# YamaneKoyo/mri-to-speech

Hardware: AMD Instinct MI355X
Metric: rtMRI frames/s end-to-end (256x256 frames -> 64-bin mel -> 11413 Hz wav) (higher is better)
Workload: dtype bf16x3; 1 GPU; e2e rtMRI->wav, 64 clips x 30 frames per GPU at 256x256 (configs[3] per-GPU share); clips_per_gpu=64, frames_per_clip=30, global_batch_clips=64, hw=256, parallelism=dp1, chunk=1920

## Files before the change

### mri-to-speech_amd/csrc/acoustic_cnn.cpp

```cpp
#include <algorithm>
#include <initializer_list>
#include <utility>

#include "plan_util.hpp"
#include "prof.hpp"

namespace m2s {

Acoustic::Acoustic(const StateDict& sd, int n_mels, int hidden, int dtype, int device)
    : dtype_(dtype), device_(device), n_mels_(n_mels), hidden_(hidden) {
  for (auto [name, v] : std::initializer_list<std::pair<const char*, bool*>>{
           {"M2S_IR_FUSED", &ir_fused_},   {"M2S_IR_WS", &ir_ws_},         {"M2S_IR_WS_S2", &ir_ws_s2_},
           {"M2S_IRWS_F32", &irws_f32_},   {"M2S_STEM_FUSED", &stem_fused_}, {"M2S_F8_EXPAND", &f8_expand_},
           {"M2S_F8_S2", &f8_s2_},         {"M2S_F8_ER", &f8_er_},         {"M2S_ER8_X8", &er8_x8_},
           {"M2S_F8_ER2", &f8_er2_},       {"M2S_SE_Y8", &se_y8_},         {"M2S_SE_FUSED", &se_fused_},
           {"M2S_ER_FUSED", &er_fused_},   {"M2S_SE_WS", &se_ws_},         {"M2S_LSTM_PERSISTENT", &lstm_persistent_},
           {"M2S_LSTM_MID", &lstm_mid_},   {"M2S_LSTM_X3", &lstm_x3_},     {"M2S_LSTM_X3G", &lstm_x3g_},
           {"M2S_SE_SP", &se_sp_},         {"M2S_ER_MRG", &er_mrg_},       {"M2S_IR_S2BAND", &ir_s2band_},
           {"M2S_ER_S2_FUSED", &er_s2_fused_}, {"M2S_SEWS_REV", &sews_rev_}})
    env_flag(name, *v);
  env_int("M2S_IRWS_MIN", irws_min_);
  env_int("M2S_SEWS_MIN", sews_min_cus_);
  pack_acoustic(sd, n_mels, hidden, dtype, arena_, p_);
  arena_.upload(device);
  for (auto& b : p_.blocks) {
    b.c1.resolve(arena_);
    if (b.type != 0) b.c2.resolve(arena_);
    if (b.type == 2) {
      b.se1.resolve(arena_);
      b.se2.resolve(arena_);
    }
  }
  p_.lstm_ih.resolve(arena_);
  M2S_HIP(hipHostMalloc(reinterpret_cast<void**>(&err_host_), sizeof(unsigned), hipHostMallocMapped | hipHostMallocCoherent));
  *err_host_ = 0;
  M2S_HIP(hipHostGetDevicePointer(reinterpret_cast<void**>(&err_dev_), err_host_, 0));
  M2S_HIP(hipMalloc(&gsync_, std::max(lstm_small_sync_bytes(), lstm_x3g_sync_bytes())));
}

Acoustic::~Acoustic() {
  if (err_host_) (void)hipHostFree(err_host_);
  if (gsync_) (void)hipFree(gsync_);
}

unsigned Acoustic::take_async_error() { return __atomic_exchange_n(err_host_, 0u, __ATOMIC_ACQ_REL); }

void Acoustic::effnet_dims(int H, int W, size_t* io, size_t* mid, size_t* se) const {
  size_t mio = 0, mmid = 0, mse = 0;
  for_each_backbone_map(H, W, [&](const BlockDef& d, const BlockMap& m) {
    if (d.type == 1) mmid = std::max(mmid, (size_t)m.oh * m.ow * chan_stride(d.mid));
    if (d.type == 2) {
// ... 81 lines not shown
}

template <typename T>
void Acoustic::effnet_cn(EffPass<T>& p, size_t k) {
  const Block& b = p_.blocks[k];
  ConvArgs a = conv2d_args(p, b.c1, p.cur, p.nxt);
  a.act = ACT_SILU;
  a.res = b.skip ? p.cur : nullptr;
  run_conv<T>(a, b.c1, p.s);
}

template <typename T>
void Acoustic::effnet_er(EffPass<T>& p, size_t k) {
  const Block& b = p_.blocks[k];
  const int nc = p.nc, oh = p.oh, ow = p.ow, nh = p.nh, nw = p.nw, qt = p.qt, ql = p.ql;
  T *const cur = p.cur, *const nxt = p.nxt;
  hipStream_t s = p.s;
  const int co = chan_stride(b.cout);
  const double px = (double)nc * nh * nw, flops = 2.0 * px * b.mid * (9.0 * b.cin + b.cout);
  auto unfused = [&] {
    ConvArgs a = conv2d_args(p, b.c1, cur, p.b.M);
    a.act = ACT_SILU;
    ConvArgs q = pw_args(b.c2, p.b.M, nxt, nc * nh * nw, nh * nw);
    q.res = b.skip ? cur : nullptr;
    if (kSplit<T> && er_s2_fused_ && b.stride == 2 && conv_gemm_er_supported(a, q)) {
      launch_conv_gemm_er(a, q, s, flops,
                          4.0 * ((double)nc * oh * ow * b.cin + px * b.cout + (9.0 * b.cin + b.cout) * b.mid));
    } else {
      run_conv<T>(a, b.c1, s);
      run_conv<T>(q, b.c2, s);
    }
  };
  if constexpr (kSplit<T>) {
    if (er_fused_ && b.er_sp && er_sp_supported(nh, nw, b.c1.cs_in, b.mid, co)) {
      launch_er_sp(cur, nc, nh, nw, b.c1.cs_in, b.mid, co, arena_.ptr(b.er_sp_w), b.c1.b, b.c2.b, nxt, flops,
                   4.0 * px * (b.c1.cs_in + co), s, er_mrg_);
    } else if (er_fused_ && b.ers_sp && b.stride == 2 && ers2_sp_supported(nh, nw, b.c1.cs_in, b.mid, co)) {
      launch_ers2_sp(cur, nc, oh, ow, nh, nw, qt, ql, b.c1.cs_in, b.mid, co, arena_.ptr(b.er_wexp), b.c1.b,
                     arena_.ptr(b.er_wpwl), b.c2.b, nxt, flops, 4.0 * ((double)nc * oh * ow * b.c1.cs_in + px * co), s);
    } else {
      unfused();
    }
  } else if constexpr (std::is_same<T, bf16_t>::value) {
    uint8_t *const cur8 = p.cur8, *const *const X8 = p.b.X8, *&next8 = p.next8;
    const Block* const nb = k + 1 < p_.blocks.size() ? &p_.blocks[k + 1] : nullptr;
    uint8_t* const er8_next = X8[0] && f8_er_ && nb && ((er8_x8_ && nb->er8) || (f8_er2_ && nb->er8w))
                                  ? (cur8 == X8[0] ? X8[1] : X8[0])
                                  : nullptr;
    if (er_fused_ && f8_er_ && b.er8 && er8_fused_supported(nh, nw, b.cin, b.mid, b.cout)) {
      uint8_t* y8 = cur8 && er8_next && er8_fused_supported(nh, nw, b.cout, b.mid, b.cout) ? er8_next : nullptr;
      launch_er8_fused(cur, nc, nh, nw, arena_.at<uint8_t>(b.er8_wexp), arena_.at<float>(b.er8_sexp), b.c1.b,
                       arena_.at<uint8_t>(b.er8_wpwl), arena_.at<float>(b.er8_spwl), b.c2.b, nxt, flops,
                       2.0 * px * (2.0 * b.cin) + (3.0 * 8 * 2048 + 2 * 2048), s, cur8, y8);
      next8 = y8;
    } else if (er_fused_ && b.er_frag && er_fused_supported(nh, nw, b.cin, b.mid, b.cout, b.c1.kp, b.c2.kp)) {
      launch_er_fused(cur, nc, nh, nw, arena_.at<bf16_t>(b.er_wexp), b.c1.b, arena_.at<bf16_t>(b.er_wpwl), b.c2.b, nxt,
                      flops, 2.0 * px * (2.0 * b.cin) + 2.0 * (9.0 * 32 * 128 + 128 * 32), s);
    } else if (er_fused_ && f8_er_ && f8_er2_ && b.er8w && cur8 &&
               er8w_fused_supported(nh, nw, b.c1.cs_in, b.mid, b.cout)) {
      uint8_t* y8 = er8_next && nb->er8w ? er8_next : nullptr;
      launch_er8w_fused(cur, cur8, nc, nh, nw, arena_.at<uint8_t>(b.er8w_w), arena_.at<float>(b.er8w_sexp), b.c1.b,
                        arena_.at<float>(b.er8w_spwl), b.c2.b, nxt, y8, flops,
                        px * (b.cin + 2.0 * b.cin + 2.0 * b.cout + (y8 ? b.cout : 0.0)) + (9.0 * b.cin + b.cout) * b.mid, s);
      next8 = y8;
    } else if (er_fused_ && b.er_frag && er2_fused_supported(nh, nw, b.c1.cs_in, b.mid, b.cout, b.c1.kp, b.c2.kp)) {
      launch_er2_fused(cur, nc, nh, nw, arena_.at<bf16_t>(b.er_wexp), b.c1.b, b.c2.b, nxt, flops,
                       2.0 * px * (2.0 * b.c1.cs_in) + 2.0 * er2_stage_elems(), s);
    } else if (er_fused_ && b.er_frag && b.stride == 2 &&
               ers2_fused_supported(nh, nw, b.c1.cs_in, b.mid, co, b.c1.kp, b.c2.kp)) {
// ... 249 lines not shown
```

### mri-to-speech_amd/csrc/er_sp_fused.hip

```cpp
#include <algorithm>

#include "kernels.hpp"
#include "lds_dma.hpp"
#include "prof.hpp"

namespace m2s {
namespace {

__device__ __forceinline__ bf16x8 frag(const char* p) { return *reinterpret_cast<const bf16x8*>(p); }
__device__ __forceinline__ f32x4 mfma(bf16x8 a, bf16x8 b, f32x4 c) {
  return __builtin_amdgcn_mfma_f32_16x16x32_bf16(a, b, c, 0, 0, 0);
}

struct ErSpArgs {
  const bf16_t* x;
  const bf16_t* wst;
  const float* bexp;
  const float* bpwl;
  bf16_t* y;
  int N, H, W, tiles_x, tiles_y;
};

template <int TH, int CSI, int NT, int ON, int NW, int MRG>
__global__ void __launch_bounds__(64 * NW, NW == 4 ? 2 : 1) er_sp_kernel(const ErSpArgs a) {
  constexpr int TW = 16, HW = TW + 2, HH = TH + 2, HPIX = HH * HW;
  constexpr int HPB = (HPIX + 63) / 64;
  constexpr int HPLANE = HPB * 1024;
  constexpr int CH = CSI / 8;
  constexpr int HBUF = 2 * CH * HPLANE;
  constexpr int HP = 2 * CH * HPB / NW;
  static_assert((2 * CH * HPB) % NW == 0, "halo pieces must divide over the waves");
  constexpr int PPW = (MRG * NT + NW - 1) / NW;
  constexpr int SLOT = PPW * NW * 1024;
  constexpr int KC = CSI / 32, NCE = 9 * KC * 2;
  constexpr int MID = NT * 16, KS = MID / 32, PN = ON * KS;
  constexpr int NPS = (PN + NT - 1) / NT;
  constexpr int NST = (NCE + 2 * NPS) / MRG;
  static_assert(MRG == 1 || (MRG == 2 && NPS == 1 && NCE % 2 == 0), "merged stages");
  constexpr int RPW = TH / NW;
  constexpr int ST = RPW * ON * 2;
  static_assert(NT % 2 == 0 && ON * 16 == CSI && TH % NW == 0, "er_sp shape");

  extern __shared__ __attribute__((aligned(16))) char smem[];
  char* ring = smem;
  char* hbuf = smem + 3 * SLOT;
  float* bexp_l = reinterpret_cast<float*>(hbuf + 2 * HBUF);
  const int tid = threadIdx.x, lane = tid & 63;
  const int wave = __builtin_amdgcn_readfirstlane(tid >> 6);
  const int g = lane >> 4, r16 = lane & 15;
  const int tpi = a.tiles_x * a.tiles_y, ntiles = a.N * tpi;

  const void* zpage = zero_page();
  auto stage_dma = [&](int ls, int slot) {
#pragma unroll
    for (int j = 0; j < PPW; ++j) {
      const int piece = wave * PPW + j;
      const void* src = piece < MRG * NT ? (const void*)(a.wst + ((size_t)(ls * MRG * NT + piece) * 64 + lane) * 8) : zpage;
      dma16(src, ring + slot * SLOT + piece * 1024);
    }
  };
  auto halo_dma = [&](int tile, char* buf) {
    const int n = tile / tpi, tr = tile - n * tpi;
    const int ty0 = (tr / a.tiles_x) * TH - 1, tx0 = (tr - (tr / a.tiles_x) * a.tiles_x) * TW - 1;
    const bf16_t* xi = a.x + (size_t)n * a.H * a.W * (2 * CSI);
#pragma unroll
    for (int j = 0; j < HP; ++j) {
      const int piece = wave * HP + j, pc = piece / HPB, pb = piece - pc * HPB;
      const int p = pb * 64 + lane, hy = p / HW, hx = p - hy * HW;
      const int iy = ty0 + hy, ix = tx0 + hx;
      const void* src = zpage;
      if (p < HPIX && iy >= 0 && iy < a.H && ix >= 0 && ix < a.W)
        src = xi + ((size_t)iy * a.W + ix) * (2 * CSI) + (pc / CH) * CSI + (pc % CH) * 8;
      dma16(src, buf + pc * HPLANE + pb * 1024);
    }
  };

  for (int i = tid; i < MID; i += 64 * NW) bexp_l[i] = a.bexp[i];
  __syncthreads();
  float4 bp[ON];
#pragma unroll
  for (int on = 0; on < ON; ++on) bp[on] = *reinterpret_cast<const float4*>(a.bpwl + on * 16 + 4 * g);

#ifndef ERSP_PRIO
#define ERSP_PRIO 1
#endif
  if (ERSP_PRIO && NW == 8 && wave >= 4) __builtin_amdgcn_s_setprio(1);
  int q = 0;
  if ((int)blockIdx.x < ntiles) {
    stage_dma(0, 0);
    stage_dma(1, 1);
    halo_dma(blockIdx.x, hbuf);
  }
  for (int it = 0, tile = blockIdx.x; tile < ntiles; tile += gridDim.x, ++it) {
    const bool has_next = tile + (int)gridDim.x < ntiles;
    const char* hb = hbuf + (it & 1) * HBUF;
    const int n = tile / tpi, tr = tile - n * tpi;
    const int oy0 = (tr / a.tiles_x) * TH, ox = (tr - (tr / a.tiles_x) * a.tiles_x) * TW + r16;

    auto begin_stage = [&](int ls) -> const char* {
      if (ls == 0) {
        if (it == 0) wait_vm<0>();
        else wait_vm<PPW + ST>();
      } else if (ls == 1) {
        if (has_next) wait_vm<ST + PPW + HP>();
        else wait_vm<ST + PPW>();
      } else if (ls == 2) {
        if (has_next) wait_vm<HP + PPW>();
        else wait_vm<PPW>();
      } else if (ls + 1 < NST || has_next) {
        wait_vm<PPW>();
      } else {
        wait_vm<0>();
      }
      __builtin_amdgcn_s_barrier();
      asm volatile("" ::: "memory");
      if (ls + 2 < NST) stage_dma(ls + 2, (q + 2) % 3);
      else if (has_next) stage_dma(ls + 2 - NST, (q + 2) % 3);
      if (ls == 0 && has_next) halo_dma(tile + gridDim.x, hbuf + ((it + 1) & 1) * HBUF);
      const char* ws = ring + (q % 3) * SLOT + lane * 16;
      ++q;
      return ws;
    };

    f32x4 acc[RPW][NT];
#pragma unroll
    for (int i = 0; i < RPW; ++i)
#pragma unroll
      for (int nt = 0; nt < NT; ++nt) acc[i][nt] = f32x4{0.f, 0.f, 0.f, 0.f};
#pragma unroll 1
    for (int ks = 0; ks < 9 * KC; ++ks) {
      const int t = ks / KC, kc = ks - t * KC, ky = t / 3, kx = t - (t / 3) * 3;
      bf16x8 bh[RPW], bl[RPW];
      const char* wsm = MRG == 2 ? begin_stage(ks) : nullptr;
      {
        const char* ws = MRG == 2 ? wsm : begin_stage(2 * ks);
#pragma unroll
        for (int i = 0; i < RPW; ++i) {
          const int pix = (RPW * wave + i + ky) * HW + r16 + kx;
          bh[i] = frag(hb + (kc * 4 + g) * HPLANE + pix * 16);
          bl[i] = frag(hb + (CH + kc * 4 + g) * HPLANE + pix * 16);
        }
#pragma unroll
        for (int nt = 0; nt < NT; ++nt) {
          const bf16x8 af = frag(ws + nt * 1024);
#pragma unroll
          for (int i = 0; i < RPW; ++i) acc[i][nt] = mfma(af, bl[i], mfma(af, bh[i], acc[i][nt]));
        }
      }
      {
        const char* ws = MRG == 2 ? wsm + NT * 1024 : begin_stage(2 * ks + 1);
#pragma unroll
        for (int nt = 0; nt < NT; ++nt) {
          const bf16x8 af = frag(ws + nt * 1024);
#pragma unroll
          for (int i = 0; i < RPW; ++i) acc[i][nt] = mfma(af, bh[i], acc[i][nt]);
        }
      }
    }

    bf16x8 mh[RPW][KS], ml[RPW][KS];
#pragma unroll
    for (int kk = 0; kk < KS; ++kk)
#pragma unroll
      for (int i = 0; i < RPW; ++i) {
        float v[8];
#pragma unroll
        for (int hh = 0; hh < 2; ++hh) {
          const int nt = 2 * kk + hh;
          const float4 bb = lds_f4(bexp_l + nt * 16 + 4 * g);
          v[4 * hh + 0] = silu(acc[i][nt][0] + bb.x);
          v[4 * hh + 1] = silu(acc[i][nt][1] + bb.y);
          v[4 * hh + 2] = silu(acc[i][nt][2] + bb.z);
          v[4 * hh + 3] = silu(acc[i][nt][3] + bb.w);
        }
        uint2 h0, l0, h1, l1;
        split4(v, h0, l0);
        split4(v + 4, h1, l1);
        mh[i][kk] = __builtin_bit_cast(bf16x8, make_uint4(h0.x, h0.y, h1.x, h1.y));
        ml[i][kk] = __builtin_bit_cast(bf16x8, make_uint4(l0.x, l0.y, l1.x, l1.y));
      }

    f32x4 o[RPW][ON];
#pragma unroll
    for (int i = 0; i < RPW; ++i)
#pragma unroll
      for (int on = 0; on < ON; ++on) o[i][on] = f32x4{0.f, 0.f, 0.f, 0.f};
    const char* wpm = MRG == 2 ? begin_stage(NCE / 2) : nullptr;
#pragma unroll
    for (int pl = 0; pl < 2; ++pl)
#pragma unroll
      for (int ps = 0; ps < NPS; ++ps) {
        const char* ws = MRG == 2 ? wpm + pl * NT * 1024 : begin_stage(NCE + pl * NPS + ps);
#pragma unroll
        for (int nt = 0; nt < NT; ++nt) {
          const int j = ps * NT + nt;
          if (j >= PN) break;
          const int kk = j / ON, on = j - (j / ON) * ON;
          const bf16x8 af = frag(ws + nt * 1024);
#pragma unroll
          for (int i = 0; i < RPW; ++i) {
            o[i][on] = mfma(af, mh[i][kk], o[i][on]);
            if (pl == 0) o[i][on] = mfma(af, ml[i][kk], o[i][on]);
          }
        }
      }

#pragma unroll
    for (int i = 0; i < RPW; ++i) {
      const int ry = RPW * wave + i, oy = oy0 + ry;
      const int cpix = ((ry + 1) * HW + r16 + 1) * 16;
#pragma unroll
      for (int on = 0; on < ON; ++on) {
        const int c4 = on * 16 + 4 * g;
        float rh[4], rl[4];
        unpack_bf16x4(lds_u2(hb + (c4 >> 3) * HPLANE + cpix + (c4 & 7) * 2), rh);
        unpack_bf16x4(lds_u2(hb + (CH + (c4 >> 3)) * HPLANE + cpix + (c4 & 7) * 2), rl);
        const float v[4] = {o[i][on][0] + bp[on].x + rh[0] + rl[0], o[i][on][1] + bp[on].y + rh[1] + rl[1],
                            o[i][on][2] + bp[on].z + rh[2] + rl[2], o[i][on][3] + bp[on].w + rh[3] + rl[3]};
        uint2 h, l;
        split4(v, h, l);
        bf16_t* yo = a.y + (((size_t)n * a.H + oy) * a.W + ox) * (2 * CSI) + c4;
        *reinterpret_cast<uint2*>(yo) = h;
        *reinterpret_cast<uint2*>(yo + CSI) = l;
      }
    }
  }
  wait_vm<0>();
}

template <int TH, int CSI, int NT, int ON, int NW, int MRG>
void launch_t(const ErSpArgs& a, const char* name, double flops, double bytes, hipStream_t s) {
  constexpr int HW = 18, HPB = ((TH + 2) * HW + 63) / 64, CH = CSI / 8, PPW = (MRG * NT + NW - 1) / NW;
  const size_t lds = 3 * (size_t)PPW * NW * 1024 + 2 * (size_t)(2 * CH * HPB * 1024) + NT * 16 * sizeof(float);
  M2S_CHECK(lds <= (NW == 4 ? 80 : 160) * 1024, "er_sp: LDS budget");
  allow_lds(reinterpret_cast<const void*>(&er_sp_kernel<TH, CSI, NT, ON, NW, MRG>));
  const int cus = device_cus();
  const int grid = std::min(a.N * a.tiles_x * a.tiles_y, (NW == 4 ? 2 : 1) * cus);
  ProfScope ps(name, flops, bytes, s);
  hipLaunchKernelGGL((er_sp_kernel<TH, CSI, NT, ON, NW, MRG>), dim3(grid), dim3(64 * NW), lds, s, a);
  M2S_HIP(hipGetLastError());
}

int tile_rows(int cs_in) { return cs_in == 32 ? 16 : 8; }

}

bool er_sp_supported(int H, int W, int cs_in, int mid, int cs_out) {
  const bool shape = (cs_in == 32 && mid == 128 && cs_out == 32) || (cs_in == 64 && mid == 224 && cs_out == 64);
  return shape && H > 0 && W > 0 && W % 16 == 0 && H % tile_rows(cs_in) == 0;
}

int er_sp_nt_stages(int cs_in, int mid, int cs_out, int* nt) {
  *nt = mid / 16;
  const int kc = cs_in / 32, pn = (cs_out / 16) * (mid / 32);
  return 9 * kc * 2 + 2 * ((pn + *nt - 1) / *nt);
}

void launch_er_sp(const void* x, int N, int H, int W, int cs_in, int mid, int cs_out, const void* wst, const float* bexp,
                  const float* bpwl, void* y, double flops, double bytes, hipStream_t s, bool merged) {
  M2S_CHECK(er_sp_supported(H, W, cs_in, mid, cs_out) && N > 0, "er_sp: unsupported shape");
  ErSpArgs a;
  a.x = static_cast<const bf16_t*>(x);
  a.wst = static_cast<const bf16_t*>(wst);
  a.bexp = bexp;
  a.bpwl = bpwl;
  a.y = static_cast<bf16_t*>(y);
  a.N = N;
  a.H = H;
  a.W = W;
  a.tiles_x = W / 16;
  a.tiles_y = H / tile_rows(cs_in);
  if (cs_in == 32 && merged)
    launch_t<16, 32, 8, 2, 8, 2>(a, "er_sp_kernel<16, 32, 8, 2, 8, 2>", flops, bytes, s);
  else if (cs_in == 32)
    launch_t<16, 32, 8, 2, 8, 1>(a, "er_sp_kernel<16, 32, 8, 2, 8, 1>", flops, bytes, s);
  else
    launch_t<8, 64, 14, 4, 8, 1>(a, "er_sp_kernel<8, 64, 14, 4, 8, 1>", flops, bytes, s);
}

}
```

### mri-to-speech_amd/csrc/kernels.hpp

```cpp
#pragma once

#include "m2s_common.hpp"

namespace m2s {

enum AsyncCode : unsigned { M2S_ASYNC_LSTM = 1u, M2S_ASYNC_WS = 2u };
struct AsyncReport {
  unsigned spin_max = 1u << 20;
  unsigned* err = nullptr;
};
__device__ __forceinline__ void report_async(unsigned* err, unsigned code, int lane) {
  if (err && lane == 0) __hip_atomic_store(err, code, __ATOMIC_RELAXED, __HIP_MEMORY_SCOPE_SYSTEM);
}

template <typename T>
void launch_stem(const float* frames, int N, int H, int W, int OH, int OW, int pad_t, int pad_l,
                 const float* w9, const float* bias, int cout, int cs_out, T* y, hipStream_t s);

int dw_pixel_blocks(int OH, int OW);
template <typename T>
void launch_dwconv(const T* x, int N, int IH, int IW, int OH, int OW, int stride, int pad_t, int pad_l,
                   int C, int cs, const float* w9, const float* bias, T* y, float* sums, hipStream_t s);

template <typename T>
// ... 64 lines not shown
int rb1_frag_taps(int C, int k, bool split);
void launch_rb1_fused(const bf16_t* x, bf16_t* s, int B, int L, int C, int k, int np, const int* dil,
                      const bf16_t* const* w1, const float* const* b1, const bf16_t* const* w2,
                      const float* const* b2, int kp, int accum, float div, bool split, double flops, double bytes,
                      hipStream_t st);

void launch_stem_b0(const float* frames, int N, int H, int W, int OH, int OW, int pad_t, int pad_l, const float* w9,
                    const float* b9, const void* w0, const float* b0, int kp0, const void* w1, const float* b1,
                    int kp1, void* y, bool split, double flops, double bytes, hipStream_t s);

bool se_excite_supported(int rd, int kp2, int cs_mid);
void launch_se_excite(const void* mean, int N, int mid, int cs_mid, const void* w1, int kp1, const float* b1,
                      int rd, const void* w2, int kp2, const float* b2, void* gate, bool split, hipStream_t s);

bool er_fused_supported(int H, int W, int cin, int mid, int cout, int kp_exp, int kp_pwl);
void launch_er_fused(const bf16_t* x, int N, int H, int W, const bf16_t* wexp, const float* bexp, const bf16_t* wpwl,
                     const float* bpwl, bf16_t* y, double flops, double bytes, hipStream_t s);

bool er8_fused_supported(int H, int W, int cin, int mid, int cout);
void launch_er8_fused(const bf16_t* x, int N, int H, int W, const uint8_t* wexp, const float* sexp, const float* bexp,
                      const uint8_t* wpwl, const float* spwl, const float* bpwl, bf16_t* y, double flops, double bytes,
                      hipStream_t s, const uint8_t* x8 = nullptr, uint8_t* y8 = nullptr);

bool er2_fused_supported(int H, int W, int cs_in, int mid, int cout, int kp_exp, int kp_pwl);
int er2_stage_elems();
bool er8w_fused_supported(int H, int W, int cs_in, int mid, int cout);
size_t er8w_stream_bytes();
void launch_er8w_fused(const bf16_t* x, const uint8_t* x8, int N, int H, int W, const uint8_t* wst, const float* sexp,
                       const float* bexp, const float* spwl, const float* bpwl, bf16_t* y, uint8_t* y8, double flops,
                       double bytes, hipStream_t s);
void launch_er2_fused(const bf16_t* x, int N, int H, int W, const bf16_t* wst, const float* bexp, const float* bpwl,
                      bf16_t* y, double flops, double bytes, hipStream_t s);

bool er_sp_supported(int H, int W, int cs_in, int mid, int cs_out);
int er_sp_nt_stages(int cs_in, int mid, int cs_out, int* nt);
void launch_er_sp(const void* x, int N, int H, int W, int cs_in, int mid, int cs_out, const void* wst, const float* bexp,
                  const float* bpwl, void* y, double flops, double bytes, hipStream_t s, bool merged = true);

bool ers2_fused_supported(int OH, int OW, int cs_in, int mid, int cs_out, int kp_exp, int kp_pwl);
int ers2_exp_elems(int cs_in, int mid);
bool ers2_sp_supported(int OH, int OW, int cs_in, int mid, int cs_out);
void launch_ers2_sp(const void* x, int N, int H, int W, int OH, int OW, int pad_t, int pad_l, int cs_in, int mid,
                    int cs_out, const void* wexp, const float* bexp, const void* wpwl, const float* bpwl, void* y,
                    double flops, double bytes, hipStream_t s);
void launch_ers2_fused(const bf16_t* x, int N, int H, int W, int OH, int OW, int pad_t, int pad_l, int cs_in, int mid,
                       int cs_out, const bf16_t* wexp, const float* bexp, const bf16_t* wpwl, const float* bpwl,
                       bf16_t* y, double flops, double bytes, hipStream_t s, uint8_t* y8 = nullptr);

void launch_preprocess(const uint8_t* frames, int N, int H, int W, int channels, float* out, hipStream_t s);

void launch_frames(const uint8_t* frames, int N, int h, int w, int channels, int out_h, int out_w, int interp, int norm,
                   float* out, hipStream_t s);

template <typename T>
void launch_gap(const T* x, int N, int P, int C, int cs, float* feats, hipStream_t s);

void launch_lstm_step(const float* pre, const float* whh, float* hs, float* cst, int B, int T, int H,
                      int step, hipStream_t s);

bool lstm_persistent_supported(int H);
size_t lstm_persistent_sync_bytes();
bool lstm_small_supported(int B, int H);
size_t lstm_small_sync_bytes();
void launch_lstm_small(const float* pre, const float* whh, float* hs, int B, int T, int H, void* sync, unsigned spin_max,
                       unsigned* err_host, hipStream_t s, unsigned* epoch = nullptr);
constexpr unsigned LSTM_SPIN_MAX = 1u << 24;
bool lstm_mid_supported(int B, int H);
size_t lstm_mid_sync_bytes();
void launch_lstm_mid(const float* pre, const float* whh, float* hs, int B, int T, int H, void* sync, unsigned spin_max,
                     unsigned* err_host, hipStream_t s);
// ... 79 lines not shown
```

### mri-to-speech_amd/csrc/model.hpp

```cpp
#pragma once

#include <map>
#include <string>
#include <vector>

#include "../../include/m2s.h"
#include "conv_igemm.hpp"
#include "kernels.hpp"

namespace m2s {

struct HostTensor {
  const float* data = nullptr;
  std::vector<int64_t> shape;
  size_t numel() const {
    size_t n = 1;
    for (auto d : shape) n *= (size_t)d;
    return n;
  }
};
using StateDict = std::map<std::string, HostTensor>;
StateDict make_state_dict(const m2s_tensor* t, int n);

class Arena {
// ... 199 lines not shown
  ~Acoustic();
  Acoustic(const Acoustic&) = delete;
  Acoustic& operator=(const Acoustic&) = delete;
  unsigned take_async_error();
  unsigned lstm_spin_max_ = LSTM_SPIN_MAX;
  unsigned ws_spin_max_ = 1u << 20;
  AsyncReport ws_report() const {
    AsyncReport r;
    r.spin_max = ws_spin_max_;
    r.err = err_dev_;
    return r;
  }
  int device() const { return device_; }
  int n_mels() const { return n_mels_; }
  int chunk = 1920;
  bool ir_fused_ = true;
  bool ir_ws_ = true;
  bool ir_ws_s2_ = true;
  int irws_min_ = 512;
  bool irws_f32_ = true;
  int sews_min_cus_ = 1;
  bool stem_fused_ = true;
  bool f8_er_ = true;
  bool se_y8_ = true;
  bool f8_er2_ = true;
  bool er8_x8_ = true;
  bool f8_expand_ = true;
  bool f8_s2_ = true;
  bool se_fused_ = true;
  bool er_fused_ = true;
  bool se_sp_ = false;
  bool se_ws_ = true;
  bool er_mrg_ = true;
  bool ir_s2band_ = true;
  bool er_s2_fused_ = true;
  bool sews_rev_ = true;
  bool lstm_persistent_ = true;
  bool lstm_mid_ = true;
  bool lstm_x3_ = true;
  bool lstm_x3g_ = true;

  size_t workspace_bytes(int B, int T, int H, int W) const;
  void forward(const float* frames, int B, int T, int H, int W, float* mel_norm, Workspace& ws, hipStream_t s);
  void effnet(const float* frames, int N, int H, int W, float* feats, int stop_after, float* probe, int* probe_dims,
              Workspace& ws, hipStream_t s);
  void bilstm(const float* feats, int B, int T, float* y, float* mel_norm, Workspace& ws, hipStream_t s);
  size_t ragged_workspace_bytes(const int* lengths, int B, int H, int W) const;
  void bilstm_ragged(const float* feats, const int* lengths, int B, long N, float* y, float* mel_norm, Workspace& ws,
                     hipStream_t s);
  void forward_ragged(const float* frames, const int* lengths, int B, long N, int H, int W, float* mel_norm,
                      Workspace& ws, hipStream_t s);
  size_t windowed_workspace_bytes(const int* lengths, const int* context, int B, int H, int W, int window,
                                  int merge) const;
  void bilstm_windowed(const float* feats, const int* lengths, const int* context, int B, long N, int window, int merge,
                       float* y, float* mel_norm, Workspace& ws, hipStream_t s);
  void forward_windowed(const float* frames, const int* lengths, const int* context, int B, long N, int H, int W,
                        int window, int merge, float* mel_norm, Workspace& ws, hipStream_t s);
  size_t pairs_workspace_bytes(const int* lengths, int B, int H, int W, int window) const;
  void bilstm_pairs(const float* feats, const int* lengths, int B, long N, int window, float* y, float* mel_norm,
                    Workspace& ws, hipStream_t s);
  void forward_pairs(const float* frames, const int* lengths, int B, long N, int H, int W, int window, float* mel_norm,
                     Workspace& ws, hipStream_t s);

 private:
  struct WindowBufs {
    int* tab = nullptr;
// ... 158 lines not shown
```

### mri-to-speech_amd/csrc/pack_acoustic.cpp

```cpp
#include <algorithm>
#include <cmath>
#include <cstring>

#include "pack.hpp"

namespace m2s {

StateDict make_state_dict(const m2s_tensor* t, int n) {
  StateDict sd;
  for (int i = 0; i < n; ++i) {
    M2S_CHECK(t[i].name != nullptr, "state dict entry without a name");
    if (t[i].elem != M2S_ELEM_F32) continue;
    M2S_CHECK(t[i].ndim >= 0 && t[i].ndim <= 4, std::string("bad ndim for ") + t[i].name);
    HostTensor h;
    h.data = static_cast<const float*>(t[i].data);
    for (int d = 0; d < t[i].ndim; ++d) h.shape.push_back(t[i].shape[d]);
    sd[t[i].name] = h;
  }
  return sd;
}

size_t Arena::add(const void* p, size_t bytes) {
  size_t off = (host_.size() + 255) & ~size_t(255);
  host_.resize(off + bytes);
// ... 161 lines not shown
  }
  const int pdt = dtype == M2S_DT_FP8 ? M2S_DT_BF16 : dtype;
  for_each_backbone_block([&](const BlockDef& d) {
    Block b{d};
    const std::string q = d.key();
    const int k = d.k, cin = d.cin;
    auto conv2d_kxk = [&](PConv& pc, const float* w, int ci, int co, const BN& bn) {
      pc = make_pconv(KIND_CONV2D, ci, co, k * k, pdt);
      pc.ks = k;
      pc.stride = b.stride;
      pc.macs_per_row = (double)co * ci * k * k;
      pack_conv(ar, pdt, pc, [&](int, int n, int t, int c) { return w[((size_t)n * ci + c) * k * k + t] * bn.a[n]; },
                [&](int n) { return bn.b[n]; });
    };
    auto conv1x1 = [&](PConv& pc, const float* w, int ci, int co, const BN& bn) {
      pc = make_pconv(KIND_GEMM, ci, co, 1, pdt);
      pc.macs_per_row = (double)co * ci;
      pack_conv(ar, pdt, pc, [&](int, int n, int, int c) { return w[(size_t)n * ci + c] * bn.a[n]; },
                [&](int n) { return bn.b[n]; });
    };
    if (b.type == 0) {
      const BN bn1 = fold_bn(sd, q + "bn1", b.cout);
      conv2d_kxk(b.c1, need(sd, q + "conv.weight", {b.cout, cin, k, k}).data, cin, b.cout, bn1);
    } else if (b.type == 1) {
      const BN e1 = fold_bn(sd, q + "bn1", b.mid);
      const float* we = need(sd, q + "conv_exp.weight", {b.mid, cin, k, k}).data;
      conv2d_kxk(b.c1, we, cin, b.mid, e1);
      const BN e2 = fold_bn(sd, q + "bn2", b.cout);
      const float* wq = need(sd, q + "conv_pwl.weight", {b.cout, b.mid, 1, 1}).data;
      conv1x1(b.c2, wq, b.mid, b.cout, e2);
      const int csi = b.c1.cs_in, cso = chan_stride(b.cout);
      const ErWeights w{we, wq, &e1, &e2, cin, csi, b.mid, b.cout, cso};
      const bool s1 = b.stride == 1 && b.skip && k == 3, s2 = b.stride == 2 && k == 3;
      if (dtype == M2S_DT_BF16X3 && s1 && er_sp_supported(32, 32, csi, b.mid, cso)) {
        pack_er_sp(ar, w, b);
      } else if (dtype == M2S_DT_BF16X3 && s2 && ers2_sp_supported(8, 16, csi, b.mid, cso)) {
        pack_ers2_fused(ar, w, true, b);
      } else if (pdt == M2S_DT_BF16 && s1 && er_fused_supported(64, 64, cin, b.mid, b.cout, b.c1.kp, b.c2.kp)) {
        pack_er_fused(ar, w, b);
        if (dtype == M2S_DT_FP8) pack_er8(ar, w, b);
      } else if (pdt == M2S_DT_BF16 && s1 && er2_fused_supported(32, 32, csi, b.mid, b.cout, b.c1.kp, b.c2.kp)) {
        pack_er2_fused(ar, w, b);
        if (dtype == M2S_DT_FP8 && er8w_fused_supported(32, 32, csi, b.mid, b.cout)) pack_er8w(ar, w, b);
      } else if (pdt == M2S_DT_BF16 && s2 && ers2_fused_supported(8, 16, csi, b.mid, cso, b.c1.kp, b.c2.kp)) {
        pack_ers2_fused(ar, w, false, b);
      }
    } else {
      const int m = b.mid, cs = chan_stride(m), rd = b.rd;
      p.max_mid_cs = std::max(p.max_mid_cs, cs);
      const BN bn1 = fold_bn(sd, q + "bn1", m);
      const float* wp = need(sd, q + "conv_pw.weight", {m, cin, 1, 1}).data;
      conv1x1(b.c1, wp, cin, m, bn1);
      if (dtype == M2S_DT_FP8 && chan_stride(cin) <= 256) {
        size_t boff = 0;
        b.f8x_kp = round_up(chan_stride(cin), 128);
        pack_gemm_f8(ar, cin, m, round_up(cs, 32), b.f8x_kp, [&](int n, int c) { return wp[(size_t)n * cin + c] * bn1.a[n]; },
                     [&](int n) { return bn1.b[n]; }, &b.f8x_w, &b.f8x_s, &boff);
        b.f8_pw = true;
      }
      const float* wd = need(sd, q + "conv_dw.weight", {m, 1, k, k}).data;
      const BN bn2 = fold_bn(sd, q + "bn2", m);
      std::vector<float> w9((size_t)cs * 9, 0.f), bd(cs, 0.f);
      for (int c = 0; c < m; ++c) {
        for (int t = 0; t < 9; ++t) w9[(size_t)t * cs + c] = wd[(size_t)c * 9 + t] * bn2.a[c];
        bd[c] = bn2.b[c];
      }
      b.dw_w = ar.add_vec(w9);
// ... 71 lines not shown
```

Baseline: 51530 rtMRI frames/s.

## Pack 56-channel K dimension in stride-1 edge-residual split-bf16 kernel

For the 64-stride, 56-real-channel edge-residual block, the 3x3 expansion GEMM's K dimension is repacked so the 9 taps x 7 channel-chunks fill 16 k-steps instead of 18. This removes the MFMA work spent on zero-padded channels. The change also uses a two-deep weight ring with a single barrier per merged stage, asm DMA issue, and scheduling hints to overlap LDS reads with MFMAs. In exchange it adds a more complex index mapping, padding-aware residual handling, and a separate unpacked kernel variant, which raises correctness risk if the weight packing layout does not match.

New measurement: 51860 rtMRI frames/s (median of 6 runs). About the same (+0.6%).

```diff
diff --git a/mri-to-speech_amd/csrc/acoustic_cnn.cpp b/mri-to-speech_amd/csrc/acoustic_cnn.cpp
--- a/mri-to-speech_amd/csrc/acoustic_cnn.cpp
+++ b/mri-to-speech_amd/csrc/acoustic_cnn.cpp
@@ -17,6 +17,7 @@
            {"M2S_ER_FUSED", &er_fused_},   {"M2S_SE_WS", &se_ws_},         {"M2S_LSTM_PERSISTENT", &lstm_persistent_},
            {"M2S_LSTM_MID", &lstm_mid_},   {"M2S_LSTM_X3", &lstm_x3_},     {"M2S_LSTM_X3G", &lstm_x3g_},
            {"M2S_SE_SP", &se_sp_},         {"M2S_ER_MRG", &er_mrg_},       {"M2S_IR_S2BAND", &ir_s2band_},
+           {"M2S_ER_KPACK", &er_kpack_},
            {"M2S_ER_S2_FUSED", &er_s2_fused_}, {"M2S_SEWS_REV", &sews_rev_}})
     env_flag(name, *v);
   env_int("M2S_IRWS_MIN", irws_min_);
@@ -164,9 +165,9 @@
     }
   };
   if constexpr (kSplit<T>) {
-    if (er_fused_ && b.er_sp && er_sp_supported(nh, nw, b.c1.cs_in, b.mid, co)) {
-      launch_er_sp(cur, nc, nh, nw, b.c1.cs_in, b.mid, co, arena_.ptr(b.er_sp_w), b.c1.b, b.c2.b, nxt, flops,
-                   4.0 * px * (b.c1.cs_in + co), s, er_mrg_);
+    if (er_fused_ && b.er_sp && er_sp_supported(nh, nw, b.cin, b.c1.cs_in, b.mid, co)) {
+      launch_er_sp(cur, nc, nh, nw, b.cin, b.c1.cs_in, b.mid, co, arena_.ptr(b.er_sp_w), b.c1.b, b.c2.b, nxt, flops,
+                   4.0 * px * (b.c1.cs_in + co), s, er_mrg_, er_kpack_);
     } else if (er_fused_ && b.ers_sp && b.stride == 2 && ers2_sp_supported(nh, nw, b.c1.cs_in, b.mid, co)) {
       launch_ers2_sp(cur, nc, oh, ow, nh, nw, qt, ql, b.c1.cs_in, b.mid, co, arena_.ptr(b.er_wexp), b.c1.b,
                      arena_.ptr(b.er_wpwl), b.c2.b, nxt, flops, 4.0 * ((double)nc * oh * ow * b.c1.cs_in + px * co), s);
diff --git a/mri-to-speech_amd/csrc/er_sp_fused.hip b/mri-to-speech_amd/csrc/er_sp_fused.hip
--- a/mri-to-speech_amd/csrc/er_sp_fused.hip
+++ b/mri-to-speech_amd/csrc/er_sp_fused.hip
@@ -21,42 +21,80 @@
   int N, H, W, tiles_x, tiles_y;
 };
 
-template <int TH, int CSI, int NT, int ON, int NW, int MRG>
-__global__ void __launch_bounds__(64 * NW, NW == 4 ? 2 : 1) er_sp_kernel(const ErSpArgs a) {
-  constexpr int TW = 16, HW = TW + 2, HH = TH + 2, HPIX = HH * HW;
-  constexpr int HPB = (HPIX + 63) / 64;
-  constexpr int HPLANE = HPB * 1024;
-  constexpr int CH = CSI / 8;
-  constexpr int HBUF = 2 * CH * HPLANE;
-  constexpr int HP = 2 * CH * HPB / NW;
-  static_assert((2 * CH * HPB) % NW == 0, "halo pieces must divide over the waves");
-  constexpr int PPW = (MRG * NT + NW - 1) / NW;
-  constexpr int SLOT = PPW * NW * 1024;
-  constexpr int KC = CSI / 32, NCE = 9 * KC * 2;
+#ifndef ERSP_KP_AHEAD
+#define ERSP_KP_AHEAD 1
+#endif
+#ifndef ERSP_KP_1BAR
+#define ERSP_KP_1BAR 1
+#endif
+template <int TH, int CSI, int NT, int ON, int NW, int MRG, bool KP>
+struct ErSpShape {
+  static constexpr int TW = 16, HW = TW + 2, HH = TH + 2, HPIX = HH * HW;
+  static constexpr int HPB = (HPIX + 63) / 64;
+  static constexpr int HPLANE = HPB * 1024;
+  static constexpr int CH = KP ? 7 : CSI / 8;
+  static constexpr int HBUF = 2 * CH * HPLANE;
+  static constexpr int HPT = 2 * CH * HPB;
+  static constexpr int HP = (HPT + NW - 1) / NW;
+  static constexpr int PPW = (MRG * NT + NW - 1) / NW;
+  static constexpr int SLOT = PPW * NW * 1024;
+  static constexpr int D = KP && MRG == 2 ? 2 : 3;
+  static constexpr int DUMP = KP ? 1024 : 0;
+  static constexpr size_t LDS = (size_t)D * SLOT + 2 * HBUF + DUMP + NT * 16 * sizeof(float);
+  static_assert(KP || HPT % NW == 0, "halo pieces must divide over the waves");
+  static_assert(!KP || (CSI == 64 && TH == NW), "K packing: 56 channels at stride 64");
+};
+
+template <int TH, int CSI, int NT, int ON, int NW, int MRG, bool KP>
+__device__ __forceinline__ void er_sp_body(const ErSpArgs a) {
+  using S = ErSpShape<TH, CSI, NT, ON, NW, MRG, KP>;
+  constexpr int TW = S::TW, HW = S::HW, HPIX = S::HPIX, HPB = S::HPB, HPLANE = S::HPLANE, CH = S::CH;
+  constexpr int HBUF = S::HBUF, HPT = S::HPT, HP = S::HP, PPW = S::PPW, SLOT = S::SLOT, D = S::D;
+  constexpr int KC = CSI / 32;
+  constexpr int NKS = KP ? 16 : 9 * KC, NCE = NKS * 2;
+  constexpr int SKIP = 9 * KC * 2 - NCE;
   constexpr int MID = NT * 16, KS = MID / 32, PN = ON * KS;
   constexpr int NPS = (PN + NT - 1) / NT;
   constexpr int NST = (NCE + 2 * NPS) / MRG;
-  static_assert(MRG == 1 || (MRG == 2 && NPS == 1 && NCE % 2 == 0), "merged stages");
+  static_assert(MRG == 1 || (MRG == 2 && (NPS == 1 || NPS == 2) && NCE % 2 == 0), "merged stages");
   constexpr int RPW = TH / NW;
   constexpr int ST = RPW * ON * 2;
   static_assert(NT % 2 == 0 && ON * 16 == CSI && TH % NW == 0, "er_sp shape");
 
   extern __shared__ __attribute__((aligned(16))) char smem[];
   char* ring = smem;
-  char* hbuf = smem + 3 * SLOT;
-  float* bexp_l = reinterpret_cast<float*>(hbuf + 2 * HBUF);
+  char* hbuf = smem + D * SLOT;
+  char* dump = hbuf + 2 * HBUF;
+  float* bexp_l = reinterpret_cast<float*>(dump + S::DUMP);
   const int tid = threadIdx.x, lane = tid & 63;
   const int wave = __builtin_amdgcn_readfirstlane(tid >> 6);
   const int g = lane >> 4, r16 = lane & 15;
   const int tpi = a.tiles_x * a.tiles_y, ntiles = a.N * tpi;
 
   const void* zpage = zero_page();
+  auto kp_dma = [&](const void* src, char* dst) {
+    if constexpr (ERSP_KP_AHEAD) dma16_asm(src, lds_lo32_u(dst));
+    else dma16(src, dst);
+  };
   auto stage_dma = [&](int ls, int slot) {
-#pragma unroll
-    for (int j = 0; j < PPW; ++j) {
-      const int piece = wave * PPW + j;
-      const void* src = piece < MRG * NT ? (const void*)(a.wst + ((size_t)(ls * MRG * NT + piece) * 64 + lane) * 8) : zpage;
-      dma16(src, ring + slot * SLOT + piece * 1024);
+    if constexpr (!KP) {
+#pragma unroll
+      for (int j = 0; j < PPW; ++j) {
+        const int piece = wave * PPW + j;
+        const void* src = piece < MRG * NT ? (const void*)(a.wst + ((size_t)(ls * MRG * NT + piece) * 64 + lane) * 8) : zpage;
+        dma16(src, ring + slot * SLOT + piece * 1024);
+      }
+    } else {
+      const int fs = ls * MRG, j = 4 * (fs >> 1) + g, t = j / 7, c = j - 7 * t;
+      const bool ce = fs < NCE, none = ce && j >= 63;
+      const size_t lane0 = ce ? ((size_t)(2 * (2 * t + (c >> 2)) + (fs & 1)) * NT * 64 + (c & 3) * 16 + r16) * 8
+                              : ((size_t)(fs + SKIP) * NT * 64 + lane) * 8;
+#pragma unroll
+      for (int jp = 0; jp < PPW; ++jp) {
+        const int piece = wave * PPW + jp;
+        const void* src = piece < MRG * NT && !none ? (const void*)(a.wst + lane0 + (size_t)piece * 64 * 8) : zpage;
+        kp_dma(src, ring + slot * SLOT + piece * 1024);
+      }
     }
   };
   auto halo_dma = [&](int tile, char* buf) {
@@ -66,12 +104,17 @@
 #pragma unroll
     for (int j = 0; j < HP; ++j) {
       const int piece = wave * HP + j, pc = piece / HPB, pb = piece - pc * HPB;
+      if (KP && piece >= HPT) {
+        kp_dma(zpage, dump);
+        continue;
+      }
       const int p = pb * 64 + lane, hy = p / HW, hx = p - hy * HW;
       const int iy = ty0 + hy, ix = tx0 + hx;
       const void* src = zpage;
       if (p < HPIX && iy >= 0 && iy < a.H && ix >= 0 && ix < a.W)
         src = xi + ((size_t)iy * a.W + ix) * (2 * CSI) + (pc / CH) * CSI + (pc % CH) * 8;
-      dma16(src, buf + pc * HPLANE + pb * 1024);
+      if constexpr (KP) kp_dma(src, buf + pc * HPLANE + pb * 1024);
+      else dma16(src, buf + pc * HPLANE + pb * 1024);
     }
   };
 
@@ -88,7 +131,7 @@
   int q = 0;
   if ((int)blockIdx.x < ntiles) {
     stage_dma(0, 0);
-    stage_dma(1, 1);
+    if (D == 3) stage_dma(1, 1);
     halo_dma(blockIdx.x, hbuf);
   }
   for (int it = 0, tile = blockIdx.x; tile < ntiles; tile += gridDim.x, ++it) {
@@ -97,8 +140,12 @@
     const int n = tile / tpi, tr = tile - n * tpi;
     const int oy0 = (tr / a.tiles_x) * TH, ox = (tr - (tr / a.tiles_x) * a.tiles_x) * TW + r16;
 
-    auto begin_stage = [&](int ls) -> const char* {
-      if (ls == 0) {
+    auto begin_stage_r = [&](int ls, auto reads) -> const char* {
+      if constexpr (D == 2) {
+        if (ls == 0 && it != 0) wait_vm<ST>();
+        else if (ls == 1 && has_next) wait_vm<HP>();
+        else wait_vm<0>();
+      } else if (ls == 0) {
         if (it == 0) wait_vm<0>();
         else wait_vm<PPW + ST>();
       } else if (ls == 1) {
@@ -114,22 +161,79 @@
       }
       __builtin_amdgcn_s_barrier();
       asm volatile("" ::: "memory");
-      if (ls + 2 < NST) stage_dma(ls + 2, (q + 2) % 3);
-      else if (has_next) stage_dma(ls + 2 - NST, (q + 2) % 3);
+      reads(ring + (q % D) * SLOT + lane * 16);
+      if (ls + D - 1 < NST) stage_dma(ls + D - 1, (q + D - 1) % D);
+      else if (has_next) stage_dma(ls + D - 1 - NST, (q + D - 1) % D);
       if (ls == 0 && has_next) halo_dma(tile + gridDim.x, hbuf + ((it + 1) & 1) * HBUF);
-      const char* ws = ring + (q % 3) * SLOT + lane * 16;
+      const char* ws = ring + (q % D) * SLOT + lane * 16;
       ++q;
       return ws;
     };
+    auto begin_stage = [&](int ls) -> const char* { return begin_stage_r(ls, [](const char*) {}); };
 
     f32x4 acc[RPW][NT];
 #pragma unroll
     for (int i = 0; i < RPW; ++i)
 #pragma unroll
       for (int nt = 0; nt < NT; ++nt) acc[i][nt] = f32x4{0.f, 0.f, 0.f, 0.f};
+    if constexpr (KP && ERSP_KP_AHEAD) {
+      static_assert(RPW == 1, "K packing: one row per wave");
 #pragma unroll 1
-    for (int ks = 0; ks < 9 * KC; ++ks) {
-      const int t = ks / KC, kc = ks - t * KC, ky = t / 3, kx = t - (t / 3) * 3;
+      for (int ks = 0; ks < NKS; ++ks) {
+        const int j = 4 * ks + g;
+        int t = j / 7, hc = j - 7 * t;
+        if (j >= 63) t = 8, hc = 0;
+        const int pix = (wave + t / 3) * HW + r16 + t - (t / 3) * 3;
+        const char* hp = hb + hc * HPLANE + pix * 16;
+        bf16x8 af[NT], al[NT], bh, bl;
+        const char* ws = begin_stage_r(MRG == 2 ? ks : 2 * ks, [&](const char* w) {
+          bh = frag(hp), bl = frag(hp + CH * HPLANE);
+#pragma unroll
+          for (int nt = 0; nt < NT; ++nt) af[nt] = frag(w + nt * 1024);
+#pragma unroll
+          for (int nt = 0; nt < 2 + NT; ++nt) __builtin_amdgcn_sched_group_barrier(0x100, 1, 0);
+        });
+#pragma unroll
+        for (int nt = 0; nt < NT; ++nt) acc[0][nt] = mfma(af[nt], bh, acc[0][nt]);
+        if constexpr (MRG == 2) {
+#pragma unroll
+          for (int nt = 0; nt < NT; ++nt) {
+            acc[0][nt] = mfma(af[nt], bl, acc[0][nt]);
+            al[nt] = frag(ws + (NT + nt) * 1024);
+          }
+#pragma unroll
+          for (int nt = 0; nt < NT; ++nt) __builtin_amdgcn_sched_group_barrier(0x008, 1, 0);
+#pragma unroll
+          for (int nt = 0; nt < NT; ++nt) {
+            __builtin_amdgcn_sched_group_barrier(0x008, 1, 0);
+            __builtin_amdgcn_sched_group_barrier(0x100, 1, 0);
+          }
+        } else {
+#pragma unroll
+          for (int nt = 0; nt < NT; ++nt) acc[0][nt] = mfma(af[nt], bl, acc[0][nt]);
+#pragma unroll
+          for (int nt = 0; nt < NT; ++nt) __builtin_amdgcn_sched_group_barrier(0x008, 1, 0);
+          begin_stage_r(2 * ks + 1, [&](const char* w) {
+#pragma unroll
+            for (int nt = 0; nt < NT; ++nt) al[nt] = frag(w + nt * 1024);
+#pragma unroll
+            for (int nt = 0; nt < NT; ++nt) __builtin_amdgcn_sched_group_barrier(0x100, 1, 0);
+          });
+        }
+#pragma unroll
+        for (int nt = 0; nt < NT; ++nt) acc[0][nt] = mfma(al[nt], bh, acc[0][nt]);
+      }
+    } else {
+#pragma unroll 1
+    for (int ks = 0; ks < NKS; ++ks) {
+      int t = ks / KC, kc = ks - t * KC;
+      if constexpr (KP) {
+        const int j = 4 * ks + g;
+        t = j / 7, kc = j - 7 * t;
+        if (j >= 63) t = 8, kc = 0;
+      }
+      const int ky = t / 3, kx = t - (t / 3) * 3;
+      const int hc = KP ? kc : kc * 4 + g;
       bf16x8 bh[RPW], bl[RPW];
       const char* wsm = MRG == 2 ? begin_stage(ks) : nullptr;
       {
@@ -137,8 +241,8 @@
 #pragma unroll
         for (int i = 0; i < RPW; ++i) {
           const int pix = (RPW * wave + i + ky) * HW + r16 + kx;
-          bh[i] = frag(hb + (kc * 4 + g) * HPLANE + pix * 16);
-          bl[i] = frag(hb + (CH + kc * 4 + g) * HPLANE + pix * 16);
+          bh[i] = frag(hb + (KP ? hc : kc * 4 + g) * HPLANE + pix * 16);
+          bl[i] = frag(hb + (KP ? CH + hc : CH + kc * 4 + g) * HPLANE + pix * 16);
         }
 #pragma unroll
         for (int nt = 0; nt < NT; ++nt) {
@@ -156,6 +260,8 @@
           for (int i = 0; i < RPW; ++i) acc[i][nt] = mfma(af, bh[i], acc[i][nt]);
         }
       }
+    }
+
     }
 
     bf16x8 mh[RPW][KS], ml[RPW][KS];
@@ -185,12 +291,14 @@
     for (int i = 0; i < RPW; ++i)
 #pragma unroll
       for (int on = 0; on < ON; ++on) o[i][on] = f32x4{0.f, 0.f, 0.f, 0.f};
-    const char* wpm = MRG == 2 ? begin_stage(NCE / 2) : nullptr;
+    const char* wpm = nullptr;
 #pragma unroll
     for (int pl = 0; pl < 2; ++pl)
 #pragma unroll
       for (int ps = 0; ps < NPS; ++ps) {
-        const char* ws = MRG == 2 ? wpm + pl * NT * 1024 : begin_stage(NCE + pl * NPS + ps);
+        const int sg = pl * NPS + ps;
+        if (MRG == 2 && sg % 2 == 0) wpm = begin_stage((NCE + sg) / 2);
+        const char* ws = MRG == 2 ? wpm + (sg % 2) * NT * 1024 : begin_stage(NCE + sg);
 #pragma unroll
         for (int nt = 0; nt < NT; ++nt) {
           const int j = ps * NT + nt;
@@ -212,9 +320,12 @@
 #pragma unroll
       for (int on = 0; on < ON; ++on) {
         const int c4 = on * 16 + 4 * g;
+        const bool pad = KP && c4 >= 56;
+        const int rc = pad ? 6 : c4 >> 3;
         float rh[4], rl[4];
-        unpack_bf16x4(lds_u2(hb + (c4 >> 3) * HPLANE + cpix + (c4 & 7) * 2), rh);
-        unpack_bf16x4(lds_u2(hb + (CH + (c4 >> 3)) * HPLANE + cpix + (c4 & 7) * 2), rl);
+        unpack_bf16x4(lds_u2(hb + rc * HPLANE + cpix + (c4 & 7) * 2), rh);
+        unpack_bf16x4(lds_u2(hb + (CH + rc) * HPLANE + cpix + (c4 & 7) * 2), rl);
+        if (pad) rh[0] = rh[1] = rh[2] = rh[3] = rl[0] = rl[1] = rl[2] = rl[3] = 0.f;
         const float v[4] = {o[i][on][0] + bp[on].x + rh[0] + rl[0], o[i][on][1] + bp[on].y + rh[1] + rl[1],
                             o[i][on][2] + bp[on].z + rh[2] + rl[2], o[i][on][3] + bp[on].w + rh[3] + rl[3]};
         uint2 h, l;
@@ -228,16 +339,30 @@
   wait_vm<0>();
 }
 
+template <int CSI, int MRG, bool KP>
+constexpr int body_mrg() { return KP && ERSP_KP_1BAR ? 2 : MRG; }
 template <int TH, int CSI, int NT, int ON, int NW, int MRG>
+__global__ void __launch_bounds__(64 * NW, NW == 4 ? 2 : 1) er_sp_kernel(const ErSpArgs a) {
+  er_sp_body<TH, CSI, NT, ON, NW, body_mrg<CSI, MRG, CSI == 64>(), CSI == 64>(a);
+}
+template <int TH, int CSI, int NT, int ON, int NW, int MRG>
+__global__ void __launch_bounds__(64 * NW, NW == 4 ? 2 : 1) er_sp_unpacked_kernel(const ErSpArgs a) {
+  er_sp_body<TH, CSI, NT, ON, NW, MRG, false>(a);
+}
+
+template <int TH, int CSI, int NT, int ON, int NW, int MRG, bool UNPACKED = false>
 void launch_t(const ErSpArgs& a, const char* name, double flops, double bytes, hipStream_t s) {
-  constexpr int HW = 18, HPB = ((TH + 2) * HW + 63) / 64, CH = CSI / 8, PPW = (MRG * NT + NW - 1) / NW;
-  const size_t lds = 3 * (size_t)PPW * NW * 1024 + 2 * (size_t)(2 * CH * HPB * 1024) + NT * 16 * sizeof(float);
-  M2S_CHECK(lds <= (NW == 4 ? 80 : 160) * 1024, "er_sp: LDS budget");
-  allow_lds(reinterpret_cast<const void*>(&er_sp_kernel<TH, CSI, NT, ON, NW, MRG>));
+  constexpr bool KP = CSI == 64 && !UNPACKED;
+  constexpr size_t lds = ErSpShape<TH, CSI, NT, ON, NW, body_mrg<CSI, MRG, KP>(), KP>::LDS;
+  static_assert(lds <= (NW == 4 ? 80 : 160) * 1024, "er_sp: LDS budget");
+  void (*kern)(const ErSpArgs);
+  if constexpr (UNPACKED) kern = &er_sp_unpacked_kernel<TH, CSI, NT, ON, NW, MRG>;
+  else kern = &er_sp_kernel<TH, CSI, NT, ON, NW, MRG>;
+  allow_lds(reinterpret_cast<const void*>(kern));
   const int cus = device_cus();
   const int grid = std::min(a.N * a.tiles_x * a.tiles_y, (NW == 4 ? 2 : 1) * cus);
   ProfScope ps(name, flops, bytes, s);
-  hipLaunchKernelGGL((er_sp_kernel<TH, CSI, NT, ON, NW, MRG>), dim3(grid), dim3(64 * NW), lds, s, a);
+  hipLaunchKernelGGL(kern, dim3(grid), dim3(64 * NW), lds, s, a);
   M2S_HIP(hipGetLastError());
 }
 
@@ -245,9 +370,9 @@
 
 }
 
-bool er_sp_supported(int H, int W, int cs_in, int mid, int cs_out) {
+bool er_sp_supported(int H, int W, int cin, int cs_in, int mid, int cs_out) {
   const bool shape = (cs_in == 32 && mid == 128 && cs_out == 32) || (cs_in == 64 && mid == 224 && cs_out == 64);
-  return shape && H > 0 && W > 0 && W % 16 == 0 && H % tile_rows(cs_in) == 0;
+  return shape && cin > 0 && cin <= cs_in && H > 0 && W > 0 && W % 16 == 0 && H % tile_rows(cs_in) == 0;
 }
 
 int er_sp_nt_stages(int cs_in, int mid, int cs_out, int* nt) {
@@ -256,9 +381,10 @@
   return 9 * kc * 2 + 2 * ((pn + *nt - 1) / *nt);
 }
 
-void launch_er_sp(const void* x, int N, int H, int W, int cs_in, int mid, int cs_out, const void* wst, const float* bexp,
-                  const float* bpwl, void* y, double flops, double bytes, hipStream_t s, bool merged) {
-  M2S_CHECK(er_sp_supported(H, W, cs_in, mid, cs_out) && N > 0, "er_sp: unsupported shape");
+void launch_er_sp(const void* x, int N, int H, int W, int cin, int cs_in, int mid, int cs_out, const void* wst,
+                  const float* bexp, const float* bpwl, void* y, double flops, double bytes, hipStream_t s, bool merged,
+                  bool kpack) {
+  M2S_CHECK(er_sp_supported(H, W, cin, cs_in, mid, cs_out) && N > 0, "er_sp: unsupported shape");
   ErSpArgs a;
   a.x = static_cast<const bf16_t*>(x);
   a.wst = static_cast<const bf16_t*>(wst);
@@ -274,8 +400,10 @@
     launch_t<16, 32, 8, 2, 8, 2>(a, "er_sp_kernel<16, 32, 8, 2, 8, 2>", flops, bytes, s);
   else if (cs_in == 32)
     launch_t<16, 32, 8, 2, 8, 1>(a, "er_sp_kernel<16, 32, 8, 2, 8, 1>", flops, bytes, s);
+  else if (kpack && cin == 56)
+    launch_t<8, 64, 14, 4, 8, 1>(a, "er_sp_kernel<8, 64, 14, 4, 8, 1>", flops, bytes, s);
   else
-    launch_t<8, 64, 14, 4, 8, 1>(a, "er_sp_kernel<8, 64, 14, 4, 8, 1>", flops, bytes, s);
-}
-
-}
+    launch_t<8, 64, 14, 4, 8, 1, true>(a, "er_sp_unpacked_kernel<8, 64, 14, 4, 8, 1>", flops, bytes, s);
+}
+
+}
diff --git a/mri-to-speech_amd/csrc/kernels.hpp b/mri-to-speech_amd/csrc/kernels.hpp
--- a/mri-to-speech_amd/csrc/kernels.hpp
+++ b/mri-to-speech_amd/csrc/kernels.hpp
@@ -120,10 +120,11 @@
 void launch_er2_fused(const bf16_t* x, int N, int H, int W, const bf16_t* wst, const float* bexp, const float* bpwl,
                       bf16_t* y, double flops, double bytes, hipStream_t s);
 
-bool er_sp_supported(int H, int W, int cs_in, int mid, int cs_out);
+bool er_sp_supported(int H, int W, int cin, int cs_in, int mid, int cs_out);
 int er_sp_nt_stages(int cs_in, int mid, int cs_out, int* nt);
-void launch_er_sp(const void* x, int N, int H, int W, int cs_in, int mid, int cs_out, const void* wst, const float* bexp,
-                  const float* bpwl, void* y, double flops, double bytes, hipStream_t s, bool merged = true);
+void launch_er_sp(const void* x, int N, int H, int W, int cin, int cs_in, int mid, int cs_out, const void* wst,
+                  const float* bexp, const float* bpwl, void* y, double flops, double bytes, hipStream_t s,
+                  bool merged = true, bool kpack = true);
 
 bool ers2_fused_supported(int OH, int OW, int cs_in, int mid, int cs_out, int kp_exp, int kp_pwl);
 int ers2_exp_elems(int cs_in, int mid);
diff --git a/mri-to-speech_amd/csrc/model.hpp b/mri-to-speech_amd/csrc/model.hpp
--- a/mri-to-speech_amd/csrc/model.hpp
+++ b/mri-to-speech_amd/csrc/model.hpp
@@ -255,6 +255,7 @@
   bool se_sp_ = false;
   bool se_ws_ = true;
   bool er_mrg_ = true;
+  bool er_kpack_ = true;
   bool ir_s2band_ = true;
   bool er_s2_fused_ = true;
   bool sews_rev_ = true;
diff --git a/mri-to-speech_amd/csrc/pack_acoustic.cpp b/mri-to-speech_amd/csrc/pack_acoustic.cpp
--- a/mri-to-speech_amd/csrc/pack_acoustic.cpp
+++ b/mri-to-speech_amd/csrc/pack_acoustic.cpp
@@ -217,7 +217,7 @@
       const int csi = b.c1.cs_in, cso = chan_stride(b.cout);
       const ErWeights w{we, wq, &e1, &e2, cin, csi, b.mid, b.cout, cso};
       const bool s1 = b.stride == 1 && b.skip && k == 3, s2 = b.stride == 2 && k == 3;
-      if (dtype == M2S_DT_BF16X3 && s1 && er_sp_supported(32, 32, csi, b.mid, cso)) {
+      if (dtype == M2S_DT_BF16X3 && s1 && er_sp_supported(32, 32, cin, csi, b.mid, cso)) {
         pack_er_sp(ar, w, b);
       } else if (dtype == M2S_DT_BF16X3 && s2 && ers2_sp_supported(8, 16, csi, b.mid, cso)) {
         pack_ers2_fused(ar, w, true, b);
```
